# zilliztech/knowhere

Measured on AMD Instinct MI355X. Metric: QPS at recall@10>=0.95, IVF-PQ 100M x d=128 batch=10k, higher is better.
Workload: dtype f32

## Files before the change

include/knhip.h:

```cpp
#ifndef KNHIP_H
#define KNHIP_H

#include <stddef.h>
#include <stdint.h>

#ifdef __cplusplus
extern "C" {
#endif

#define KNHIP_ABI_VERSION 9

typedef struct knhip_index knhip_index;

typedef enum knhip_kind {
    KNHIP_BRUTE_FORCE = 0,
    KNHIP_IVF_FLAT = 1,
    KNHIP_IVF_PQ = 2,
    KNHIP_IVF_SQ8 = 3
} knhip_kind;

typedef enum knhip_metric { KNHIP_L2 = 0, KNHIP_IP = 1 } knhip_metric;

typedef enum knhip_status {
    KNHIP_OK = 0,
// ... 225 lines not shown
enum {
    KNHIP_STAGE_COARSE = 0,
    KNHIP_STAGE_GROUP = 1,
    KNHIP_STAGE_LUT = 2,
    KNHIP_STAGE_SCAN = 3,
    KNHIP_STAGE_MERGE = 4,
    KNHIP_STAGE_OTHER = 5,
    KNHIP_STAGE_SCAN_RANK0 = 6,
    KNHIP_STAGE_TABLES = 7,
    KNHIP_STAGE_REFINE = 8,
    KNHIP_STAGE_TIES = 9
};
int knhip_profile_enable(knhip_index* idx, int on);
int knhip_profile_reset(knhip_index* idx);
int knhip_profile_get(const knhip_index* idx, knhip_stage_times* out);
const char* knhip_stage_kernel_name(int stage, int kind);

#ifdef __cplusplus
}
#endif
#endif
```

knowhere_amd/_lib.py:

```python
import ctypes as C
import os

_HERE = os.path.dirname(os.path.abspath(__file__))
LIB_PATH = os.environ.get("KNHIP_LIB") or os.path.join(_HERE, "libknhip.so")

BRUTE_FORCE, IVF_FLAT, IVF_PQ, IVF_SQ8 = 0, 1, 2, 3
L2, IP = 0, 1
NSTAGE = 16
ABI_VERSION = 9
(STAGE_COARSE, STAGE_GROUP, STAGE_LUT, STAGE_SCAN, STAGE_MERGE, STAGE_OTHER, STAGE_SCAN_RANK0, STAGE_TABLES, STAGE_REFINE,
 STAGE_TIES) = range(10)
STAGE_NAMES = ["coarse", "group", "lut", "scan", "merge", "other", "scan_rank0", "tables", "refine", "ties"]


class KnhipError(RuntimeError):
    def __init__(self, code, msg):
        super().__init__(f"knhip error {code}: {msg}")
        self.code = code


class Desc(C.Structure):
    _fields_ = [("kind", C.c_int32), ("metric", C.c_int32), ("dim", C.c_int32), ("device", C.c_int32),
                ("nlist", C.c_int64), ("pq_m", C.c_int32), ("pq_nbits", C.c_int32),
                ("precomputed_table_max_bytes", C.c_int64)]


class StageTimes(C.Structure):
    _fields_ = [("ms", C.c_float * NSTAGE), ("launches", C.c_int64 * NSTAGE), ("scan_bytes", C.c_double),
                ("coarse_flops", C.c_double), ("scan_items", C.c_int64), ("coarse_fallback_queries", C.c_int64), ("scan_bytes_rank0", C.c_double),
                ("mscan_queries", C.c_int64), ("mscan_overflow_queries", C.c_int64), ("mscan_candidates", C.c_int64), ("mscan_stream_bytes", C.c_double),
                ("mscan_recomputed", C.c_int64), ("pq_filter_form", C.c_int64), ("tie_queries", C.c_int64),
                ("tie_anomalies", C.c_int64)]


SYMBOLS = [
    "knhip_abi_version", "knhip_device_count", "knhip_last_error", "knhip_index_create",
    "knhip_index_destroy", "knhip_index_set_coarse", "knhip_index_set_pq", "knhip_index_set_sq", "knhip_index_set_sq_type", "knhip_index_get_sq_type", "knhip_index_set_row_scale", "knhip_index_add_assigned_by", "knhip_index_get_desc",
    "knhip_index_add_lists", "knhip_index_add_vectors", "knhip_index_set_coarse_device",
    "knhip_index_set_lists_device", "knhip_index_add_vectors_device", "knhip_index_count",
    "knhip_index_device_bytes", "knhip_index_uses_precomputed_table", "knhip_index_last_range_ranks", "knhip_search",
    "knhip_search_device", "knhip_coarse_search_device", "knhip_merge_topk_device",
    "knhip_search_canonical_device", "knhip_ties_rule_applies", "knhip_tie_flag_device", "knhip_tie_arrivals_device", "knhip_tie_resolve_device",
    "knhip_tie_flag_host", "knhip_tie_resolve_host", "knhip_refine_distances_device", "knhip_refine_rows_distances_device",
    "knhip_refine_combine_device", "knhip_refine_select_device", "knhip_refine_select_host",
    "knhip_merge_topk_host", "knhip_refine_device", "knhip_fvec_L2sqr_ny", "knhip_fvec_inner_products_ny",
    "knhip_fvec_norms_L2sqr", "knhip_fvec_madd", "knhip_int8_vec_L2sqr_ny",
    "knhip_int8_vec_inner_products_ny", "knhip_profile_enable", "knhip_profile_reset",
    "knhip_profile_get", "knhip_stage_kernel_name", "knhip_range_search", "knhip_range_search_ranked", "knhip_free", "knhip_search_preassigned_device",
    "knhip_kmeans_device", "knhip_index_train", "knhip_index_train_device", "knhip_index_add", "knhip_index_add_device",
    "knhip_index_encode_device", "knhip_index_get_coarse", "knhip_index_get_pq", "knhip_index_get_sq",
    "knhip_index_get_list_sizes", "knhip_index_get_lists", "knhip_index_get_vectors_device", "knhip_search_refine",
    "knhip_index_get_vectors", "knhip_index_find_vectors", "knhip_index_assign", "knhip_device_memory",
    "knhip_rows_create", "knhip_rows_destroy", "knhip_rows_train", "knhip_rows_train_uniform", "knhip_rows_set_trained", "knhip_rows_get_trained",
    "knhip_rows_add", "knhip_rows_add_codes", "knhip_rows_get_codes", "knhip_rows_count", "knhip_rows_code_size",
    "knhip_rows_device_bytes", "knhip_search_refine_rows", "knhip_refine_rows_device",
# ... 58 lines not shown
    L.knhip_index_set_sq.argtypes = [vp, vp, vp]
    L.knhip_index_set_sq_type.argtypes = [vp, i32]
    L.knhip_index_get_sq_type.argtypes = [vp]
    L.knhip_index_get_sq_type.restype = i32
    L.knhip_index_set_row_scale.argtypes = [vp, vp, i32]
    L.knhip_index_add_assigned_by.argtypes = [vp, i64, vp, vp, vp]
    L.knhip_index_add_lists.argtypes = [vp, vp, vp, vp]
    L.knhip_index_set_lists_device.argtypes = [vp, vp, vp, vp]
    L.knhip_index_add_vectors.argtypes = [vp, i64, vp, vp, i64]
    L.knhip_index_add_vectors_device.argtypes = [vp, i64, vp, vp, i64]
    L.knhip_index_count.argtypes = [vp]
    L.knhip_index_device_bytes.argtypes = [vp]
    L.knhip_index_uses_precomputed_table.argtypes = [vp]
    L.knhip_index_last_range_ranks.argtypes = [vp]
    L.knhip_index_last_range_ranks.restype = C.c_int64
    L.knhip_search.argtypes = [vp, vp, i64, i32, i32, vp, i64, vp, vp]
    L.knhip_search_device.argtypes = [vp, vp, i64, i32, i32, vp, i64, vp, vp, vp]
    L.knhip_coarse_search_device.argtypes = [vp, vp, i64, i32, vp, vp, vp]
    L.knhip_search_preassigned_device.argtypes = [vp, vp, i64, i32, i32, vp, vp, vp, i64, vp, vp, vp]
    L.knhip_merge_topk_device.argtypes = [i32, i64, i32, i32, vp, vp, vp, vp, vp]
    L.knhip_merge_topk_host.argtypes = [i32, i64, i32, i32, vp, vp, vp, vp]
    L.knhip_refine_device.argtypes = [i32, i32, vp, i64, i64, vp, i64, vp, i32, i32, vp, vp, vp]
    L.knhip_search_canonical_device.argtypes = [vp, vp, i64, i32, i32, vp, vp, vp, i64, vp, vp, vp]
    L.knhip_tie_flag_device.argtypes = [vp, vp, i64, i32, vp, vp, vp, C.POINTER(C.c_int32), vp]
    L.knhip_tie_arrivals_device.argtypes = [vp, vp, vp, i32, vp, i32, i32, vp, vp, vp, i64, i64, vp, vp, vp, vp, vp]
    L.knhip_tie_resolve_device.argtypes = [i32, i32, vp, i32, i32, vp, vp, vp, vp, vp, vp, vp, vp, vp]
    L.knhip_tie_flag_host.argtypes = [vp, vp, i64, i32, vp, vp, vp]
    L.knhip_tie_resolve_host.argtypes = [i32, i32, i64, i32, vp, vp, vp, vp, vp, vp, vp, vp, vp]
    L.knhip_refine_distances_device.argtypes = [i32, i32, vp, i64, i64, vp, i64, vp, i32, vp, vp]
    L.knhip_refine_rows_distances_device.argtypes = [i32, vp, i64, vp, i64, vp, i32, vp, vp]
# ... 64 lines not shown
```

knowhere_amd/csrc/kernels.h:

```cpp
#pragma once

#include <hip/hip_runtime.h>
#include <stdint.h>
#include <algorithm>
#include "sq_codec.h"

namespace knhip {

struct KnItem {
    int32_t list;
    int32_t npair;
    int64_t pair0;
};
struct KnPair {
    int32_t q;
    int32_t slot;
};

__host__ __device__ constexpr int pq_stream_phase(int lane) {
    const int l = lane & 31;
    return l < 4 ? l : l < 12 ? l + 4 : l < 16 ? l - 8 : l < 20 ? l - 16 : l < 28 ? l - 12 : l - 24;
}
constexpr int PQ_STREAM_PHASES = 16;
__host__ __device__ constexpr uint32_t pq_stream_mask(int j) {
// ... 198 lines not shown
    const uint4* pq_codes_i;
    const void* pq_qi;
    const float* pq_qis;
    P16Rec* pq_recs16;
    int32_t* pq_ctr;
    int32_t pq_prune_mu;
    const void* pq_cb16;
    const void* pq_qh16;
    const float* pq_qd;
    const float* pq_sc;
    const float* pq_psum_s;
    unsigned char* pq_spill;
    int32_t pq_spill_cap;
    int32_t pq_spill_wgs;
    const int2* pq_unit_tiles;
};

int64_t pq_stream16r_blocks(int64_t len);
hipError_t launch_pq_stream16r(const uint8_t* codes, const int64_t* list_row_off, const int64_t* list_len,
                               const int64_t* list_sblk_off, int64_t nlist, uint4* out, hipStream_t s);
hipError_t launch_pq_psum(const uint8_t* codes, const int64_t* list_row_off, const int64_t* list_len,
                          const int64_t* list_sblk_off, int64_t nlist, const float* precomp_t, float* psum,
                          uint32_t* pabs_max_bits, hipStream_t s);
hipError_t launch_pqf_query_table(const float* queries, const float4* cb_m, int d, int64_t nq, bool is_l2, float pabs_max,
                                  void* qh, float* qs, hipStream_t s);
hipError_t launch_pqf_predict(const float* dump, int64_t stride, const int32_t* n_row, const float* gthr, const float* qs,
                              const float* qs2, const int64_t* keys, int nprobe, int64_t nlist, const int64_t* list_len,
                              int64_t nq, int cap, int k, bool is_l2, int32_t* poor, hipStream_t s);
size_t pqf_smem();
hipError_t launch_pq_stream16i(const uint8_t* codes, const int64_t* list_row_off, const int64_t* list_len,
// ... 79 lines not shown
    return std::max<int64_t>(groups, std::min<int64_t>(by_cost, by_tiles));
}
hipError_t launch_mscan_flat(const MScanArgs& a, bool is_l2, int64_t units_bound, hipStream_t s);
int mscan_flat_bf16_qt(int nstep);
size_t mscan_flat_bf16_smem(int nstep);
hipError_t launch_mscan_flat_bf16(const MScanArgs& a, bool is_l2, int64_t units_bound, hipStream_t s);
hipError_t launch_mscan_sq8(const MScanArgs& a, bool is_l2, int64_t units_bound, hipStream_t s);
hipError_t launch_ms_sample_plan(const int64_t* keys, int64_t nq, int nprobe, int64_t nlist, const int64_t* list_len,
                                 int smin, int cap, int32_t* sample_off, int32_t* n_row, hipStream_t s);
hipError_t launch_ms_sq8_query_prep(const float* queries, int64_t nq, int d, int ldq, const float* trained, void* qh,
                                    void* ql, float* qs, hipStream_t s, int bits = 8);
hipError_t launch_ms_tau(const float* sel_d, int64_t nq, int k, bool is_l2, float* gthr, uint2* gmeta, hipStream_t s);
hipError_t launch_mscan_finish(const MScanArgs& a, int kind, bool is_l2, const int64_t* keys, const float* coarse_dis,
                               int nprobe, int k, float* out_d, int64_t* out_i, unsigned long long* counters, int pass,
                               hipStream_t s);
hipError_t launch_ms_flag_pairs(const int32_t* overflow, int want, const int64_t* keys, int64_t nq, int nprobe,
                                int64_t nlist, const int64_t* list_len, int k, KnItem* items, KnPair* pairs,
                                int64_t* nitems, int64_t* empty_mark, hipStream_t s);

hipError_t launch_sq_scan(const SqScanArgs& a, bool is_l2, int64_t grid, hipStream_t s, int qg_override = 0);
hipError_t launch_sq_interleave(const uint8_t* codes, const int64_t* list_row_off,
                                const int64_t* list_len, const int64_t* list_blk_off, int64_t nlist,
                                int64_t code_size, uint4* out, hipStream_t s);

struct WorkTable {
    int32_t* list_count;
    int64_t* list_pair_off;
    int64_t* list_item_off;
    int32_t* list_cursor;
    KnPair* pairs;
// ... 204 lines not shown
```

knowhere_amd/csrc/knhip_api.hip:

```cpp
#include "knhip_internal.h"

namespace knhip_host {

thread_local std::string g_last_error;

int fail(int code, const std::string& msg) {
    g_last_error = msg;
    return code;
}

int build_coarse_layout(knhip_index* idx) {
    const int nchunk = (idx->d + 3) / 4;
    const int64_t nblk = (idx->nlist + 63) / 64;
    HIP_TRY(idx->centroids_il.alloc((size_t)nblk * nchunk * 64 * sizeof(float4)));
    HIP_TRY(launch_interleave_rows(idx->centroids.as<float>(), idx->nlist, idx->d,
                                   idx->centroids_il.as<float4>(), 0, nullptr));
    HIP_TRY(idx->cnorm.alloc((size_t)idx->nlist * sizeof(float)));
    HIP_TRY(launch_row_norms(idx->centroids.as<float>(), idx->nlist, idx->d, idx->cnorm.as<float>(), nullptr));
    HIP_TRY(idx->centroids_bs.alloc((size_t)idx->nlist * coarse_bf16_slabs(idx->d) * 128));
    HIP_TRY(launch_coarse_bf16_split(idx->centroids.as<float>(), idx->nlist, idx->d, idx->centroids_bs.p, nullptr));
    HIP_TRY(hipDeviceSynchronize());
    std::vector<float> cn((size_t)idx->nlist);
    HIP_TRY(hipMemcpy(cn.data(), idx->cnorm.p, cn.size() * sizeof(float), hipMemcpyDeviceToHost));
    idx->cnorm_max = cn.empty() ? 0.f : *std::max_element(cn.begin(), cn.end());
// ... 767 lines not shown
        }
        const int qt0 = mscan_queries_per_unit(kind, true);
        const int64_t units_bound = round_up(npairs / qt + std::min<int64_t>(nlist, npairs) + 1, 8);
        const int64_t sample = mscan_sample_rows();
        const int64_t np0 = std::min<int64_t>(npairs, nq * std::min<int64_t>(nprobe, sample));
        const int64_t bound0 = round_up(np0 / qt0 + std::min<int64_t>(nlist, np0) + 1, 8);
        HIP_TRY(ws->ms_units.reserve((size_t)std::max(units_bound, bound0) * sizeof(KnItem)));
        HIP_TRY(ws->ms_unit_off.reserve((size_t)(nlist + 1) * sizeof(int64_t)));
        HIP_TRY(ws->ms_nunits.reserve(sizeof(int64_t) + 2 * sizeof(double)));
        HIP_TRY(ws->ms_cand.reserve((size_t)nq * ms_cap * sizeof(int64_t)));
        HIP_TRY(ws->ms_cand_pess.reserve((size_t)nq * ms_cap * sizeof(float)));
        if (kind == KNHIP_IVF_SQ8) {
            HIP_TRY(ws->ms_eps_max.reserve((size_t)nq * sizeof(uint32_t)));
            HIP_TRY(hipMemsetAsync(ws->ms_eps_max.p, 0, (size_t)nq * sizeof(uint32_t), s));
        }
        HIP_TRY(ws->ms_cand_cnt.reserve((size_t)(2 * nq + 4) * sizeof(int32_t)));
        HIP_TRY(ws->dump.reserve((size_t)nq * sample * sizeof(float)));
        HIP_TRY(ws->sel_keys.reserve((size_t)nq * k * sizeof(int64_t)));
        HIP_TRY(ws->sel_d.reserve((size_t)nq * k * sizeof(float)));
        HIP_TRY(ws->ghist.reserve((size_t)nq * 64 * sizeof(uint32_t)));
        HIP_TRY(ws->gmeta.reserve((size_t)nq * sizeof(uint2)));
        int32_t* cand_cnt = ws->ms_cand_cnt.as<int32_t>();
        int32_t* overflow = cand_cnt + nq;
        MScanArgs m{};
        m.rows = idx->rows.p;
        m.xnorm = idx->xnorm.as<float>();
        m.xnorm_max = idx->xnorm_max;
        m.list_blk_off = idx->d_list_blk_off.as<int64_t>();
        m.list_len = idx->d_list_len.as<int64_t>();
        m.list_row_off = idx->d_list_row_off.as<int64_t>();
        m.ids = idx->ids.as<int64_t>();
// ... 327 lines not shown
        {
            StageTimer t(idx, s, KNHIP_STAGE_SCAN);
            HIP_TRY(launch_filter(m, std::max(units_bound, pqd_bound)));
        }
        {
            StageTimer t(idx, s, KNHIP_STAGE_MERGE);
            unsigned long long* counters = idx->coarse_fail_dev.as<unsigned long long>() + 1;
            MScanArgs mf = m;
            if (pq_i8) {
                mf.pq_qs = m.pq_qis;
                mf.pq_prune_mu = 1;
            }
            if (pq_dec) {
                mf.pq_qs = m.pq_qd;
            }
            HIP_TRY(launch_mscan_finish(mf, kind, is_l2, keys_p, cdis_p, nprobe, k, d_out_d, d_out_i, counters, 1, s));
            HIP_TRY(launch_ms_flag_pairs(overflow, 2, keys_p, nq, nprobe, nlist, idx->d_list_len.as<int64_t>(), k,
                                         ws->items.as<KnItem>(), wt.pairs, wt.nitems, nullptr, s));
            MScanArgs r = m;
            r.pairs = wt.pairs;
            r.units = ws->items.as<KnItem>();
            r.nunits_dev = wt.nitems;
            r.unit_loop = 1;
            r.pq_unit_tiles = nullptr;
            r.ghist = nullptr;
            r.gmeta = nullptr;
            HIP_TRY(launch_filter(r, npairs));
            HIP_TRY(launch_mscan_finish(mf, kind, is_l2, keys_p, cdis_p, nprobe, k, d_out_d, d_out_i, counters, 2, s));
            HIP_TRY(launch_ms_flag_pairs(overflow, 1, keys_p, nq, nprobe, nlist, idx->d_list_len.as<int64_t>(), k,
                                         ws->items.as<KnItem>(), wt.pairs, wt.nitems, ws->partial_i.as<int64_t>(), s));
// ... 672 lines not shown
    if (!out) {
        return fail(KNHIP_ERR_INVALID_ARGS, "get_desc: null output");
    }
    *out = idx->desc;
    return KNHIP_OK;
}

int64_t knhip_index_device_bytes(const knhip_index* idx) {
    return idx ? idx->device_bytes() : 0;
}

int64_t knhip_index_last_range_ranks(const knhip_index* idx) {
    return idx ? idx->last_range_ranks : -1;
}

int knhip_index_uses_precomputed_table(const knhip_index* idx) {
    return idx ? idx->use_precomp : 0;
}


int knhip_search_device(const knhip_index* idx, const float* d_queries, int64_t nq, int32_t k,
                        int32_t nprobe, const uint8_t* d_bitset, int64_t bitset_nbits,
                        int64_t* d_out_ids, float* d_out_dist, void* stream) {
    if (int rc = check_index(idx)) return rc;
    if (int rc = validate_search(idx, nq, k, nprobe)) return rc;
    if (nq == 0) {
        return KNHIP_OK;
    }
    if (!d_queries || !d_out_ids || !d_out_dist) {
        return fail(KNHIP_ERR_INVALID_ARGS, "null query/output pointer");
// ... 717 lines not shown
```

knowhere_amd/csrc/knhip_env.h:

```cpp
#pragma once
#include <algorithm>
#include <cstdlib>
#include <cstring>

namespace knhip_host {

struct EnvLayout {
    bool coarse_given;
    int coarse_gemm;
    size_t aos_keep_bytes;
    bool rank0_select;
    bool cand_hist;
    int pq_q4;
    int mscan;
    bool flat_bf16;
    int mscan_cap;
    int pqd_spill_cap;
    int pqf;
    bool pqf_guard;
    int pqf_form;
    bool pq_v1;
    bool bf_exact;
    int pq_waves;
};

struct EnvSearch {
    int ms_sample_rows;
    int pq_sample_rows;
    bool no_side_stream;
    bool guard_sync;
    bool range_no_waves;
    bool ties_canonical;
    bool ties_trace;
    int pqd_unit_cost;
};
constexpr int KNHIP_PQD_UNIT_COST_DEFAULT = 512;

inline bool env_is(const char* v, const char* what) { return v != nullptr && std::strcmp(v, what) == 0; }
inline int env_digit(const char* v, int lo, int hi, int dflt) { return (v && v[0] >= '0' + lo && v[0] <= '0' + hi) ? v[0] - '0' : dflt; }
inline int env_count(const char* v) { return (v && *v) ? std::max(0, std::atoi(v)) : 0; }

inline EnvLayout env_layout() {
    EnvLayout e{};
    const char* c = std::getenv("KNHIP_COARSE");
    e.coarse_given = c != nullptr;
    e.coarse_gemm = env_is(c, "exact") ? 0 : env_is(c, "fp32") ? 1 : 2;
    const char* keep = std::getenv("KNHIP_AOS_KEEP_MB");
    e.aos_keep_bytes = (keep && *keep) ? (size_t)std::max<long long>(0, std::atoll(keep)) << 20 : (size_t)8 << 30;
    const char* r0 = std::getenv("KNHIP_RANK0");
// ... 21 lines not shown

inline EnvSearch env_search() {
    EnvSearch e{};
    const char* a = std::getenv("KNHIP_MS_SAMPLE_ROWS");
    e.ms_sample_rows = a ? std::max(1, std::atoi(a)) : 0;
    const char* b = std::getenv("KNHIP_PQ_SAMPLE_ROWS");
    e.pq_sample_rows = b ? std::max(1, std::atoi(b)) : 0;
    e.no_side_stream = std::getenv("KNHIP_NO_SIDE_STREAM") != nullptr;
    e.guard_sync = std::getenv("KNHIP_PQF_GUARD_SYNC") != nullptr;
    e.range_no_waves = std::getenv("KNHIP_RANGE_NO_WAVES") != nullptr;
    const char* t = std::getenv("KNHIP_TIES");
    e.ties_canonical = t && (t[0] == 'c' || t[0] == 'C' || t[0] == '0');
    e.ties_trace = std::getenv("KNHIP_TIES_TRACE") != nullptr;
    const char* uc = std::getenv("KNHIP_PQD_UNIT_COST");
    e.pqd_unit_cost = (uc && *uc) ? std::max(0, std::atoi(uc)) : KNHIP_PQD_UNIT_COST_DEFAULT;
    return e;
}

}
```

knowhere_amd/csrc/mfma_scan.hip:

```cpp
#include "common.h"
#include "kernels.h"
#include "ms_common.h"

namespace knhip {

typedef float ms_f32x16 __attribute__((ext_vector_type(16)));
typedef _Float16 ms_f16x8 __attribute__((ext_vector_type(8)));

constexpr int MS_WAVES = 4;
constexpr int MS_THREADS = MS_WAVES * KN_WAVE;
constexpr int MS_NQT = 2;
constexpr int MS_QT = 32 * MS_NQT;
constexpr int MS_SAMPLE = 8192;

__global__ void ms_block_norms_kernel(const float4* __restrict__ rows, int64_t total_blk, int nchunk,
                                      float* __restrict__ out, float* __restrict__ out_max) {
    const int64_t t = (int64_t)blockIdx.x * blockDim.x + threadIdx.x;
    float acc = 0.f;
    if (t < total_blk * 64) {
        const int64_t b = t >> 6;
        const int r = (int)(t & 63);
        const float4* p = rows + b * (int64_t)nchunk * 64 + r;
        for (int c = 0; c < nchunk; c++) {
            const float4 v = p[(int64_t)c * 64];
// ... 964 lines not shown
        return hipSuccess;
    }
    if (is_l2) {
        hipLaunchKernelGGL(ms_tau_kernel<true>, dim3((unsigned)((nq + 255) / 256)), dim3(256), 0, s, sel_d, nq, k, gthr,
                           gmeta);
    } else {
        hipLaunchKernelGGL(ms_tau_kernel<false>, dim3((unsigned)((nq + 255) / 256)), dim3(256), 0, s, sel_d, nq, k, gthr,
                           gmeta);
    }
    return hipGetLastError();
}

constexpr int MF_THREADS = 256;
constexpr int MF_MLP = 8;

template <bool IS_L2, int KIND, int BITS = 8>
__global__ __launch_bounds__(MF_THREADS) void mscan_finish_kernel(MScanArgs a, const int64_t* __restrict__ keys,
                                                                  const float* __restrict__ coarse_dis, int nprobe,
                                                                  int k, int P_max, float* __restrict__ out_d,
                                                                  int64_t* __restrict__ out_i,
                                                                  unsigned long long* __restrict__ counters, int pass) {
    extern __shared__ __align__(16) unsigned char smem[];
    __shared__ float tab[256];
    static_assert(KIND == 3 || BITS == 8, "the code width belongs to the IVF-SQ finish");
    const int64_t q = blockIdx.x;
    const int tid = threadIdx.x;
    const int flag = a.overflow[q];
    const bool retry_prep = pass == 1 && flag == 1;
    if ((pass == 1 && flag != 0 && flag != 1) || (pass == 2 && flag != 2)) {
        if (pass == 2 && flag == 1 && tid == 0) {
            atomicAdd(counters + 1, 1ull);
        }
        return;
    }
    const int d = a.d;
    int n = min(a.cand_cnt[q], a.cap);
    const int n_filter = n;
    constexpr int MF_PRUNE_PER_THREAD = 16;
    const int n_head = min(n, MF_THREADS * MF_PRUNE_PER_THREAD);
    if ((KIND != 3 || a.eps_max != nullptr) && a.cand_pess != nullptr && !retry_prep && n >= 2 * k &&
        n_head <= MF_THREADS * MF_PRUNE_PER_THREAD) {
        __shared__ int s_cnt;
        __shared__ float s_red[MF_THREADS / KN_WAVE];
        float cmax = 0.f;
        for (int sl = tid; KIND == 2 && sl < nprobe; sl += MF_THREADS) {
            cmax = fmaxf(cmax, fabsf(coarse_dis[q * nprobe + sl]));
        }
#pragma unroll
        for (int dlt = KN_WAVE / 2; dlt > 0; dlt >>= 1) {
// ... 75 lines not shown
                if (tot >= k) {
                    hi = mid;
                } else {
                    lo = mid + 1;
                }
            }
        }
        const float tau2 = dist_key_inv<IS_L2>(lo);
        float tau_abs = fmaxf(gthr_abs, fabsf(tau2));
        if (KIND == 2 && n_head < n && a.gmeta != nullptr) {
            const uint2 mt = a.gmeta[q];
            if (mt.y != KN_HIST_OFF) {
                tau_abs = fmaxf(tau_abs, fabsf(dist_key_inv<IS_L2>(mt.x)));
            }
        }
        float eps_max = eps_q + 64.0f * 5.9604645e-8f * (cmax + tau_abs + eps_mu);
        if (KIND == 1) {
            const float qn = a.qnorm[q];
            eps_max = a.eps_scale * (IS_L2 ? (qn + a.xnorm_max) : sqrtf(qn * a.xnorm_max)) + 1e-30f;
        }
        if (KIND == 3) {
            eps_max = __uint_as_float(a.eps_max[q]);
        }
        if (eps_max < INFINITY && tau2 == tau2 && fabsf(tau2) < FLT_MAX) {
            if (tid == 0) {
                s_cnt = 0;
            }
            __syncthreads();
#pragma unroll
            for (int u = 0; u < MF_PRUNE_PER_THREAD; u++) {
                const int ci = tid + u * MF_THREADS;
                const bool keep = ci < n_head && (IS_L2 ? (pp[u] - 2.0f * eps_max <= tau2) : (pp[u] + 2.0f * eps_max >= tau2));
                if (keep) {
                    const int j = atomicAdd(&s_cnt, 1);
                    a.cand[q * (int64_t)a.cap + j] = pc[u];
                }
            }
#pragma unroll 1
            for (int ci0 = n_head; ci0 < n; ci0 += MF_THREADS) {
                const int ci = ci0 + tid;
                int64_t c = 0;
                float p = worst_dist<IS_L2>();
                if (ci < n) {
                    c = a.cand[q * (int64_t)a.cap + ci];
                    p = a.cand_pess[q * (int64_t)a.cap + ci];
                }
                __syncthreads();
                if (ci < n && (IS_L2 ? (p - 2.0f * eps_max <= tau2) : (p + 2.0f * eps_max >= tau2))) {
                    const int j = atomicAdd(&s_cnt, 1);
                    a.cand[q * (int64_t)a.cap + j] = c;
                }
            }
            __syncthreads();
            n = s_cnt;
            __syncthreads();
        }
    }
    if (retry_prep && n < k) {
        if (tid == 0) {
            atomicAdd(counters + 1, 1ull);
            a.overflow[q] = 3;
        }
        return;
// ... 62 lines not shown
                                    acc = l2_step(acc, x.x, y.x);
                                    acc = l2_step(acc, x.y, y.y);
                                    acc = l2_step(acc, x.z, y.z);
                                    acc = l2_step(acc, x.w, y.w);
                                } else {
                                    acc = ip_step(acc, x.x, y.x);
                                    acc = ip_step(acc, x.y, y.y);
                                    acc = ip_step(acc, x.z, y.z);
                                    acc = ip_step(acc, x.w, y.w);
                                }
                            }
                        }
                    }
                } else if (KIND == 2) {
                    const uint4* cp = reinterpret_cast<const uint4*>(a.pq_codes + (a.list_row_off[list] + pos) * 32);
                    const uint4 cw[2] = {cp[0], cp[1]};
                    const uint32_t ww[8] = {cw[0].x, cw[0].y, cw[0].z, cw[0].w, cw[1].x, cw[1].y, cw[1].z, cw[1].w};
                    const float* cen = a.centroids + list * d;
#pragma unroll 16
                    for (int m = 0; m < 32; m++) {
                        const int code = (int)((ww[m >> 2] >> (8 * (m & 3))) & 0xffu);
                        const float4 y = a.pq_cb_t[code * 32 + m];
                        float4 x = *reinterpret_cast<const float4*>(sq + m * 4);
                        float t;
                        if (a.pq_lut_mode == PQ_LUT_RESIDUAL) {
                            const float4 cl = *reinterpret_cast<const float4*>(cen + m * 4);
                            x = make_float4(fsub_x(x.x, cl.x), fsub_x(x.y, cl.y), fsub_x(x.z, cl.z), fsub_x(x.w, cl.w));
                            t = l2_step(0.f, x.x, y.x);
                            t = l2_step(t, x.y, y.y);
                            t = l2_step(t, x.z, y.z);
                            t = l2_step(t, x.w, y.w);
                        } else {
                            t = ip_step(0.f, x.x, y.x);
                            t = ip_step(t, x.y, y.y);
                            t = ip_step(t, x.z, y.z);
                            t = ip_step(t, x.w, y.w);
                            if (a.pq_lut_mode == PQ_LUT_PRECOMP) {
                                const float4 cl = *reinterpret_cast<const float4*>(cen + m * 4);
                                float nrm = ip_step(0.f, y.x, y.x);
                                nrm = ip_step(nrm, y.y, y.y);
                                nrm = ip_step(nrm, y.z, y.z);
                                nrm = ip_step(nrm, y.w, y.w);
                                float ipc = ip_step(0.f, cl.x, y.x);
                                ipc = ip_step(ipc, cl.y, y.y);
                                ipc = ip_step(ipc, cl.z, y.z);
                                ipc = ip_step(ipc, cl.w, y.w);
                                const float t2 = fadd_x(nrm, fmul_x(2.0f, ipc));
                                t = fadd_x(t2, fmul_x(-2.0f, t));
                            }
                        }
                        acc = fadd_x(acc, t);
                    }
                    if (a.pq_lut_mode != PQ_LUT_RESIDUAL) {
                        acc = fadd_x(coarse_dis[q * nprobe + slot], acc);
                    }
                } else if (BITS != 8) {
                    constexpr int GC = SW::GROUP_CHUNKS, GD = SW::GROUP_DIMS;
                    constexpr int NG = BITS == 6 ? 2 : 4;
                    const uint4* p = reinterpret_cast<const uint4*>(a.rows) + blk * (int64_t)a.nchunk * 64 + r;
                    const float* cen = a.centroids + list * d;
                    for (int g0 = 0; g0 < sq_ngroup; g0 += NG) {
                        uint4 wv[NG * GC];
#pragma unroll
                        for (int u = 0; u < NG * GC; u++) {
                            wv[u] = p[(int64_t)min(g0 * GC + u, a.nchunk - 1) * 64];
                        }
#pragma unroll
                        for (int gu = 0; gu < NG; gu++) {
                            const int g = g0 + gu;
                            if (g < sq_ngroup) {
// ... 98 lines not shown
        }
        return;
    }
    for (int e = tid; e < k; e += MF_THREADS) {
        float dd = worst_dist<IS_L2>();
        int64_t ii = -1;
        if (!(key[e] == 0xffffffffu && tie[e] == ~0ull)) {
            dd = dist_key_inv<IS_L2>(key[e]);
            ii = (int64_t)(IS_L2 ? tie[e] : ~tie[e]);
        }
        out_d[q * k + e] = dd;
        out_i[q * k + e] = ii;
    }
    if (pass == 2 && tid == 0) {
        a.overflow[q] = 0;
    }
}

__global__ void ms_flag_pairs_kernel(const int32_t* __restrict__ overflow, int want, const int64_t* __restrict__ keys,
                                     int64_t nq, int nprobe, int64_t nlist, const int64_t* __restrict__ list_len, int k,
                                     KnItem* __restrict__ items, KnPair* __restrict__ pairs, int64_t* __restrict__ nitems,
                                     int64_t* __restrict__ empty_mark) {
    if (overflow[nq] == 0) {
        return;
    }
    const int64_t t = (int64_t)blockIdx.x * blockDim.x + threadIdx.x;
    if (t >= nq * nprobe) {
        return;
    }
    const int64_t q = t / nprobe;
// ... 136 lines not shown
    if (kind == 1) {
        if (is_l2) MF_LAUNCH(true, 1); else MF_LAUNCH(false, 1);
    } else if (kind == 2) {
        if (is_l2) MF_LAUNCH(true, 2); else MF_LAUNCH(false, 2);
    } else if (bits == 8) {
        if (is_l2) MF_LAUNCH(true, 3); else MF_LAUNCH(false, 3);
    } else if (bits == 6) {
        if (is_l2) MF_LAUNCH(true, 3, 6); else MF_LAUNCH(false, 3, 6);
    } else {
        if (is_l2) MF_LAUNCH(true, 3, 4); else MF_LAUNCH(false, 3, 4);
    }
#undef MF_LAUNCH
    return hipGetLastError();
}

}
```

knowhere_amd/index.py:

```python
import ctypes as C

import numpy as np

from . import _lib
from ._lib import KnhipError, check

BRUTE_FORCE, IVF_FLAT, IVF_PQ, IVF_SQ8 = _lib.BRUTE_FORCE, _lib.IVF_FLAT, _lib.IVF_PQ, _lib.IVF_SQ8
L2, IP = _lib.L2, _lib.IP

KIND_NAMES = {"GPU_HIP_BRUTE_FORCE": BRUTE_FORCE, "GPU_HIP_IVF_FLAT": IVF_FLAT, "GPU_HIP_IVF_PQ": IVF_PQ,
              "GPU_HIP_IVF_SQ8": IVF_SQ8}


def _np_ptr(a):
    return None if a is None else C.c_void_p(a.ctypes.data)


def _t_ptr(t):
    return None if t is None else C.c_void_p(t.data_ptr())


def _bitset_nbits(bitset, nbits):
    if bitset is None:
        return 0
# ... 208 lines not shown
        I = np.empty((nq, k), np.int64)
        bs = None if bitset is None else np.ascontiguousarray(bitset, np.uint8)
        nbits = _bitset_nbits(bs, nbits)
        check(self.L.knhip_search_refine_rows(self.h, rows.h, _np_ptr(xq), nq, k, k_base, nprobe, _np_ptr(bs), nbits,
                                              _np_ptr(I), _np_ptr(D)))
        return D, I

    def get_vectors(self, ids):
        ids = np.ascontiguousarray(ids, np.int64)
        out = np.empty((len(ids), self.dim), np.float32)
        check(self.L.knhip_index_get_vectors(self.h, len(ids), _np_ptr(ids), _np_ptr(out)))
        return out

    def last_range_ranks(self):
        return int(self.L.knhip_index_last_range_ranks(self.h))

    def range_search(self, xq, radius, max_empty_result_buckets=2, bitset=None, nbits=0):
        xq = np.ascontiguousarray(xq, np.float32)
        nq = xq.shape[0]
        lims = np.zeros(nq + 1, np.int64)
        pi, pd = C.POINTER(C.c_int64)(), C.POINTER(C.c_float)()
        bs = None if bitset is None else np.ascontiguousarray(bitset, np.uint8)
        nbits = _bitset_nbits(bs, nbits)
        check(self.L.knhip_range_search(self.h, _np_ptr(xq), nq, float(radius), int(max_empty_result_buckets),
                                        _np_ptr(bs), nbits, _np_ptr(lims), C.byref(pi), C.byref(pd)))
        n = int(lims[-1])
        ids = np.ctypeslib.as_array(pi, shape=(n,)).copy() if n else np.empty(0, np.int64)
        dis = np.ctypeslib.as_array(pd, shape=(n,)).copy() if n else np.empty(0, np.float32)
        self.L.knhip_free(pi)
        self.L.knhip_free(pd)
# ... 348 lines not shown
```

Before: 1.564 million.

## Add wave-per-query PQ finish kernel ahead of block finish pass

Adds a new finish kernel for IVF-PQ in which each 64-lane wave handles one query. It does ballot-based threshold pruning, exact PQ recomputation of the survivors and a rank-based top-k, all inside the wave. Queries it completes are marked done, and the existing block-per-query finish kernel skips them. The aim is to stop spending a whole 256-thread block and block-level syncs on queries with few candidates. The cost is an extra launch plus a fallback path for queries that overflow the wave kernel's limits.

Result: slower. 1.492 million (-4.6%).

```diff
diff --git a/include/knhip.h b/include/knhip.h
--- a/include/knhip.h
+++ b/include/knhip.h
@@ -263,6 +263,7 @@
 int knhip_profile_enable(knhip_index* idx, int on);
 int knhip_profile_reset(knhip_index* idx);
 int knhip_profile_get(const knhip_index* idx, knhip_stage_times* out);
+int64_t knhip_index_finish_wave_queries(const knhip_index* idx);
 const char* knhip_stage_kernel_name(int stage, int kind);
 
 #ifdef __cplusplus
diff --git a/knowhere_amd/_lib.py b/knowhere_amd/_lib.py
--- a/knowhere_amd/_lib.py
+++ b/knowhere_amd/_lib.py
@@ -38,7 +38,7 @@
     "knhip_index_destroy", "knhip_index_set_coarse", "knhip_index_set_pq", "knhip_index_set_sq", "knhip_index_set_sq_type", "knhip_index_get_sq_type", "knhip_index_set_row_scale", "knhip_index_add_assigned_by", "knhip_index_get_desc",
     "knhip_index_add_lists", "knhip_index_add_vectors", "knhip_index_set_coarse_device",
     "knhip_index_set_lists_device", "knhip_index_add_vectors_device", "knhip_index_count",
-    "knhip_index_device_bytes", "knhip_index_uses_precomputed_table", "knhip_index_last_range_ranks", "knhip_search",
+    "knhip_index_device_bytes", "knhip_index_uses_precomputed_table", "knhip_index_last_range_ranks", "knhip_index_finish_wave_queries", "knhip_search",
     "knhip_search_device", "knhip_coarse_search_device", "knhip_merge_topk_device",
     "knhip_search_canonical_device", "knhip_ties_rule_applies", "knhip_tie_flag_device", "knhip_tie_arrivals_device", "knhip_tie_resolve_device",
     "knhip_tie_flag_host", "knhip_tie_resolve_host", "knhip_refine_distances_device", "knhip_refine_rows_distances_device",
@@ -127,6 +127,8 @@
     L.knhip_index_uses_precomputed_table.argtypes = [vp]
     L.knhip_index_last_range_ranks.argtypes = [vp]
     L.knhip_index_last_range_ranks.restype = C.c_int64
+    L.knhip_index_finish_wave_queries.argtypes = [vp]
+    L.knhip_index_finish_wave_queries.restype = C.c_int64
     L.knhip_search.argtypes = [vp, vp, i64, i32, i32, vp, i64, vp, vp]
     L.knhip_search_device.argtypes = [vp, vp, i64, i32, i32, vp, i64, vp, vp, vp]
     L.knhip_coarse_search_device.argtypes = [vp, vp, i64, i32, vp, vp, vp]
diff --git a/knowhere_amd/csrc/kernels.h b/knowhere_amd/csrc/kernels.h
--- a/knowhere_amd/csrc/kernels.h
+++ b/knowhere_amd/csrc/kernels.h
@@ -236,6 +236,7 @@
     int32_t pq_spill_cap;
     int32_t pq_spill_wgs;
     const int2* pq_unit_tiles;
+    const int32_t* finish_done;
 };
 
 int64_t pq_stream16r_blocks(int64_t len);
@@ -345,6 +346,10 @@
 hipError_t launch_mscan_finish(const MScanArgs& a, int kind, bool is_l2, const int64_t* keys, const float* coarse_dis,
                                int nprobe, int k, float* out_d, int64_t* out_i, unsigned long long* counters, int pass,
                                hipStream_t s);
+bool mscan_finish_wave_supports(const MScanArgs& a, int kind, int k);
+hipError_t launch_mscan_finish_wave(const MScanArgs& a, int kind, bool is_l2, const int64_t* keys,
+                                    const float* coarse_dis, int nprobe, int k, float* out_d, int64_t* out_i,
+                                    unsigned long long* counters, int32_t* done, hipStream_t s);
 hipError_t launch_ms_flag_pairs(const int32_t* overflow, int want, const int64_t* keys, int64_t nq, int nprobe,
                                 int64_t nlist, const int64_t* list_len, int k, KnItem* items, KnPair* pairs,
                                 int64_t* nitems, int64_t* empty_mark, hipStream_t s);
diff --git a/knowhere_amd/csrc/knhip_api.hip b/knowhere_amd/csrc/knhip_api.hip
--- a/knowhere_amd/csrc/knhip_api.hip
+++ b/knowhere_amd/csrc/knhip_api.hip
@@ -805,7 +805,7 @@
             HIP_TRY(ws->ms_eps_max.reserve((size_t)nq * sizeof(uint32_t)));
             HIP_TRY(hipMemsetAsync(ws->ms_eps_max.p, 0, (size_t)nq * sizeof(uint32_t), s));
         }
-        HIP_TRY(ws->ms_cand_cnt.reserve((size_t)(2 * nq + 4) * sizeof(int32_t)));
+        HIP_TRY(ws->ms_cand_cnt.reserve((size_t)(3 * nq + 4) * sizeof(int32_t)));
         HIP_TRY(ws->dump.reserve((size_t)nq * sample * sizeof(float)));
         HIP_TRY(ws->sel_keys.reserve((size_t)nq * k * sizeof(int64_t)));
         HIP_TRY(ws->sel_d.reserve((size_t)nq * k * sizeof(float)));
@@ -1163,6 +1163,12 @@
             if (pq_dec) {
                 mf.pq_qs = m.pq_qd;
             }
+            if (!env.finish_block && mscan_finish_wave_supports(mf, kind, k)) {
+                int32_t* done = ws->ms_cand_cnt.as<int32_t>() + 2 * nq + 4;
+                HIP_TRY(launch_mscan_finish_wave(mf, kind, is_l2, keys_p, cdis_p, nprobe, k, d_out_d, d_out_i, counters,
+                                                 done, s));
+                mf.finish_done = done;
+            }
             HIP_TRY(launch_mscan_finish(mf, kind, is_l2, keys_p, cdis_p, nprobe, k, d_out_d, d_out_i, counters, 1, s));
             HIP_TRY(launch_ms_flag_pairs(overflow, 2, keys_p, nq, nprobe, nlist, idx->d_list_len.as<int64_t>(), k,
                                          ws->items.as<KnItem>(), wt.pairs, wt.nitems, nullptr, s));
@@ -1865,6 +1871,19 @@
     return idx ? idx->last_range_ranks : -1;
 }
 
+int64_t knhip_index_finish_wave_queries(const knhip_index* idx) {
+    if (check_index(idx) != KNHIP_OK) {
+        return -1;
+    }
+    DeviceGuard g(idx->desc.device);
+    unsigned long long n = 0;
+    if (hipDeviceSynchronize() != hipSuccess ||
+        hipMemcpy(&n, idx->coarse_fail_dev.as<unsigned long long>() + 6, sizeof(n), hipMemcpyDeviceToHost) != hipSuccess) {
+        return -1;
+    }
+    return (int64_t)n;
+}
+
 int knhip_index_uses_precomputed_table(const knhip_index* idx) {
     return idx ? idx->use_precomp : 0;
 }
diff --git a/knowhere_amd/csrc/knhip_env.h b/knowhere_amd/csrc/knhip_env.h
--- a/knowhere_amd/csrc/knhip_env.h
+++ b/knowhere_amd/csrc/knhip_env.h
@@ -33,6 +33,7 @@
     bool ties_canonical;
     bool ties_trace;
     int pqd_unit_cost;
+    bool finish_block;
 };
 constexpr int KNHIP_PQD_UNIT_COST_DEFAULT = 512;
 
@@ -84,6 +85,7 @@
     e.ties_trace = std::getenv("KNHIP_TIES_TRACE") != nullptr;
     const char* uc = std::getenv("KNHIP_PQD_UNIT_COST");
     e.pqd_unit_cost = (uc && *uc) ? std::max(0, std::atoi(uc)) : KNHIP_PQD_UNIT_COST_DEFAULT;
+    e.finish_block = env_is(std::getenv("KNHIP_FINISH"), "block");
     return e;
 }
 
diff --git a/knowhere_amd/csrc/mfma_scan.hip b/knowhere_amd/csrc/mfma_scan.hip
--- a/knowhere_amd/csrc/mfma_scan.hip
+++ b/knowhere_amd/csrc/mfma_scan.hip
@@ -1002,6 +1002,58 @@
 constexpr int MF_THREADS = 256;
 constexpr int MF_MLP = 8;
 
+__device__ __forceinline__ float mf_pq_exact(const MScanArgs& a, const float* sq, const uint4 cw0, const uint4 cw1,
+                                             const float* __restrict__ cen, const float* __restrict__ cd) {
+    const uint32_t ww[8] = {cw0.x, cw0.y, cw0.z, cw0.w, cw1.x, cw1.y, cw1.z, cw1.w};
+    float acc = 0.f;
+#pragma unroll 16
+    for (int m = 0; m < 32; m++) {
+        const int code = (int)((ww[m >> 2] >> (8 * (m & 3))) & 0xffu);
+        const float4 y = a.pq_cb_t[code * 32 + m];
+        float4 x = *reinterpret_cast<const float4*>(sq + m * 4);
+        float t;
+        if (a.pq_lut_mode == PQ_LUT_RESIDUAL) {
+            const float4 cl = *reinterpret_cast<const float4*>(cen + m * 4);
+            x = make_float4(fsub_x(x.x, cl.x), fsub_x(x.y, cl.y), fsub_x(x.z, cl.z), fsub_x(x.w, cl.w));
+            t = l2_step(0.f, x.x, y.x);
+            t = l2_step(t, x.y, y.y);
+            t = l2_step(t, x.z, y.z);
+            t = l2_step(t, x.w, y.w);
+        } else {
+            t = ip_step(0.f, x.x, y.x);
+            t = ip_step(t, x.y, y.y);
+            t = ip_step(t, x.z, y.z);
+            t = ip_step(t, x.w, y.w);
+            if (a.pq_lut_mode == PQ_LUT_PRECOMP) {
+                const float4 cl = *reinterpret_cast<const float4*>(cen + m * 4);
+                float nrm = ip_step(0.f, y.x, y.x);
+                nrm = ip_step(nrm, y.y, y.y);
+                nrm = ip_step(nrm, y.z, y.z);
+                nrm = ip_step(nrm, y.w, y.w);
+                float ipc = ip_step(0.f, cl.x, y.x);
+                ipc = ip_step(ipc, cl.y, y.y);
+                ipc = ip_step(ipc, cl.z, y.z);
+                ipc = ip_step(ipc, cl.w, y.w);
+                const float t2 = fadd_x(nrm, fmul_x(2.0f, ipc));
+                t = fadd_x(t2, fmul_x(-2.0f, t));
+            }
+        }
+        acc = fadd_x(acc, t);
+    }
+    if (a.pq_lut_mode != PQ_LUT_RESIDUAL) {
+        acc = fadd_x(*cd, acc);
+    }
+    return acc;
+}
+
+__device__ __forceinline__ float mf_pq_eps_max(float eps_q, float cmax, float tau_abs, float eps_mu) {
+    return eps_q + 64.0f * 5.9604645e-8f * (cmax + tau_abs + eps_mu);
+}
+template <bool IS_L2>
+__device__ __forceinline__ bool mf_prune_keep(float p, float eps_max, float tau2) {
+    return IS_L2 ? (p - 2.0f * eps_max <= tau2) : (p + 2.0f * eps_max >= tau2);
+}
+
 template <bool IS_L2, int KIND, int BITS = 8>
 __global__ __launch_bounds__(MF_THREADS) void mscan_finish_kernel(MScanArgs a, const int64_t* __restrict__ keys,
                                                                   const float* __restrict__ coarse_dis, int nprobe,
@@ -1021,6 +1073,9 @@
         }
         return;
     }
+    if (pass == 1 && a.finish_done != nullptr && a.finish_done[q] != 0) {
+        return;
+    }
     const int d = a.d;
     int n = min(a.cand_cnt[q], a.cap);
     const int n_filter = n;
@@ -1126,7 +1181,7 @@
                 tau_abs = fmaxf(tau_abs, fabsf(dist_key_inv<IS_L2>(mt.x)));
             }
         }
-        float eps_max = eps_q + 64.0f * 5.9604645e-8f * (cmax + tau_abs + eps_mu);
+        float eps_max = mf_pq_eps_max(eps_q, cmax, tau_abs, eps_mu);
         if (KIND == 1) {
             const float qn = a.qnorm[q];
             eps_max = a.eps_scale * (IS_L2 ? (qn + a.xnorm_max) : sqrtf(qn * a.xnorm_max)) + 1e-30f;
@@ -1142,7 +1197,7 @@
 #pragma unroll
             for (int u = 0; u < MF_PRUNE_PER_THREAD; u++) {
                 const int ci = tid + u * MF_THREADS;
-                const bool keep = ci < n_head && (IS_L2 ? (pp[u] - 2.0f * eps_max <= tau2) : (pp[u] + 2.0f * eps_max >= tau2));
+                const bool keep = ci < n_head && mf_prune_keep<IS_L2>(pp[u], eps_max, tau2);
                 if (keep) {
                     const int j = atomicAdd(&s_cnt, 1);
                     a.cand[q * (int64_t)a.cap + j] = pc[u];
@@ -1158,7 +1213,7 @@
                     p = a.cand_pess[q * (int64_t)a.cap + ci];
                 }
                 __syncthreads();
-                if (ci < n && (IS_L2 ? (p - 2.0f * eps_max <= tau2) : (p + 2.0f * eps_max >= tau2))) {
+                if (ci < n && mf_prune_keep<IS_L2>(p, eps_max, tau2)) {
                     const int j = atomicAdd(&s_cnt, 1);
                     a.cand[q * (int64_t)a.cap + j] = c;
                 }
@@ -1251,46 +1306,7 @@
                     }
                 } else if (KIND == 2) {
                     const uint4* cp = reinterpret_cast<const uint4*>(a.pq_codes + (a.list_row_off[list] + pos) * 32);
-                    const uint4 cw[2] = {cp[0], cp[1]};
-                    const uint32_t ww[8] = {cw[0].x, cw[0].y, cw[0].z, cw[0].w, cw[1].x, cw[1].y, cw[1].z, cw[1].w};
-                    const float* cen = a.centroids + list * d;
-#pragma unroll 16
-                    for (int m = 0; m < 32; m++) {
-                        const int code = (int)((ww[m >> 2] >> (8 * (m & 3))) & 0xffu);
-                        const float4 y = a.pq_cb_t[code * 32 + m];
-                        float4 x = *reinterpret_cast<const float4*>(sq + m * 4);
-                        float t;
-                        if (a.pq_lut_mode == PQ_LUT_RESIDUAL) {
-                            const float4 cl = *reinterpret_cast<const float4*>(cen + m * 4);
-                            x = make_float4(fsub_x(x.x, cl.x), fsub_x(x.y, cl.y), fsub_x(x.z, cl.z), fsub_x(x.w, cl.w));
-                            t = l2_step(0.f, x.x, y.x);
-                            t = l2_step(t, x.y, y.y);
-                            t = l2_step(t, x.z, y.z);
-                            t = l2_step(t, x.w, y.w);
-                        } else {
-                            t = ip_step(0.f, x.x, y.x);
-                            t = ip_step(t, x.y, y.y);
-                            t = ip_step(t, x.z, y.z);
-                            t = ip_step(t, x.w, y.w);
-                            if (a.pq_lut_mode == PQ_LUT_PRECOMP) {
-                                const float4 cl = *reinterpret_cast<const float4*>(cen + m * 4);
-                                float nrm = ip_step(0.f, y.x, y.x);
-                                nrm = ip_step(nrm, y.y, y.y);
-                                nrm = ip_step(nrm, y.z, y.z);
-                                nrm = ip_step(nrm, y.w, y.w);
-                                float ipc = ip_step(0.f, cl.x, y.x);
-                                ipc = ip_step(ipc, cl.y, y.y);
-                                ipc = ip_step(ipc, cl.z, y.z);
-                                ipc = ip_step(ipc, cl.w, y.w);
-                                const float t2 = fadd_x(nrm, fmul_x(2.0f, ipc));
-                                t = fadd_x(t2, fmul_x(-2.0f, t));
-                            }
-                        }
-                        acc = fadd_x(acc, t);
-                    }
-                    if (a.pq_lut_mode != PQ_LUT_RESIDUAL) {
-                        acc = fadd_x(coarse_dis[q * nprobe + slot], acc);
-                    }
+                    acc = mf_pq_exact(a, sq, cp[0], cp[1], a.centroids + list * d, coarse_dis + q * nprobe + slot);
                 } else if (BITS != 8) {
                     constexpr int GC = SW::GROUP_CHUNKS, GD = SW::GROUP_DIMS;
                     constexpr int NG = BITS == 6 ? 2 : 4;
@@ -1419,6 +1435,232 @@
     }
     if (pass == 2 && tid == 0) {
         a.overflow[q] = 0;
+    }
+}
+
+constexpr int MFW_WAVES = 4;
+constexpr int MFW_PER_LANE = 16;
+constexpr int MFW_MAX_N = KN_WAVE * MFW_PER_LANE;
+constexpr int MFW_MAX_K = 128;
+constexpr int MFW_MAX_SURV = 256;
+constexpr int MFW_DQ = 128;
+constexpr int MFW_LDS_WAVE = MFW_MAX_SURV * 12 + MFW_DQ * 4;
+
+__device__ __forceinline__ void mfw_wave_sync() {
+    __builtin_amdgcn_fence(__ATOMIC_RELEASE, "wavefront");
+    __builtin_amdgcn_wave_barrier();
+    __builtin_amdgcn_fence(__ATOMIC_ACQUIRE, "wavefront");
+}
+
+template <bool IS_L2, int KIND>
+__global__ __launch_bounds__(MFW_WAVES * KN_WAVE, 4) void mscan_finish_wave_kernel(
+    MScanArgs a, const int64_t* __restrict__ keys, const float* __restrict__ coarse_dis, int nprobe, int k,
+    float* __restrict__ out_d, int64_t* __restrict__ out_i, unsigned long long* __restrict__ counters,
+    int32_t* __restrict__ done) {
+    extern __shared__ __align__(16) unsigned char smem[];
+    static_assert(KIND == 2, "the wave finish recomputes PQ codes; the other kinds stay on the block kernel");
+    const int lane = threadIdx.x & (KN_WAVE - 1);
+    const int wave = __builtin_amdgcn_readfirstlane((int)(threadIdx.x / KN_WAVE));
+    const int64_t q = (int64_t)blockIdx.x * MFW_WAVES + wave;
+    if (q >= a.nq) {
+        return;
+    }
+    const int n = min(a.cand_cnt[q], a.cap);
+    if (a.overflow[q] != 0 || n > MFW_MAX_N) {
+        if (lane == 0) {
+            done[q] = 0;
+        }
+        return;
+    }
+    unsigned char* my = smem + (size_t)wave * MFW_LDS_WAVE;
+    unsigned long long* tie = reinterpret_cast<unsigned long long*>(my);
+    uint32_t* key = reinterpret_cast<uint32_t*>(my + MFW_MAX_SURV * 8);
+    float* sq = reinterpret_cast<float*>(my + MFW_MAX_SURV * 12);
+    const int d = a.d;
+    for (int i = lane; i < MFW_DQ; i += KN_WAVE) {
+        sq[i] = (i < d) ? a.queries[q * d + i] : 0.f;
+    }
+    const bool have_pess = a.cand_pess != nullptr;
+    int64_t pc[MFW_PER_LANE];
+    float pp[MFW_PER_LANE];
+#pragma unroll
+    for (int u = 0; u < MFW_PER_LANE; u++) {
+        const int ci = lane + u * KN_WAVE;
+        pc[u] = 0;
+        pp[u] = worst_dist<IS_L2>();
+        if (u * KN_WAVE < n && ci < n) {
+            pc[u] = a.cand[q * (int64_t)a.cap + ci];
+            if (have_pess) {
+                pp[u] = a.cand_pess[q * (int64_t)a.cap + ci];
+            }
+        }
+    }
+    bool pruned = false;
+    float tau2 = 0.f, eps_max = 0.f;
+    if (have_pess && n >= 2 * k) {
+        float cmax = 0.f;
+        for (int sl = lane; sl < nprobe; sl += KN_WAVE) {
+            cmax = fmaxf(cmax, fabsf(coarse_dis[q * nprobe + sl]));
+        }
+        uint32_t kmn = 0xffffffffu, kmx = 0u;
+#pragma unroll
+        for (int u = 0; u < MFW_PER_LANE; u++) {
+            if (lane + u * KN_WAVE < n) {
+                const uint32_t pk = dist_key<IS_L2>(pp[u]);
+                kmn = min(kmn, pk);
+                kmx = max(kmx, pk);
+            }
+        }
+#pragma unroll
+        for (int dlt = KN_WAVE / 2; dlt > 0; dlt >>= 1) {
+            cmax = fmaxf(cmax, __shfl_xor(cmax, dlt, KN_WAVE));
+            kmn = min(kmn, (uint32_t)__shfl_xor((int)kmn, dlt, KN_WAVE));
+            kmx = max(kmx, (uint32_t)__shfl_xor((int)kmx, dlt, KN_WAVE));
+        }
+        uint32_t lo = kmn, hi = kmx;
+        while (lo < hi) {
+            const uint32_t mid = lo + ((hi - lo) >> 1);
+            int c = 0;
+#pragma unroll
+            for (int u = 0; u < MFW_PER_LANE; u++) {
+                if (u * KN_WAVE < n) {
+                    c += __popcll(__ballot(lane + u * KN_WAVE < n && dist_key<IS_L2>(pp[u]) <= mid));
+                }
+            }
+            if (c >= k) {
+                hi = mid;
+            } else {
+                lo = mid + 1;
+            }
+        }
+        tau2 = dist_key_inv<IS_L2>(lo);
+        const float eps_q = a.pq_qs[q * 4 + 2];
+        const float eps_mu = a.pq_prune_mu ? fabsf(a.pq_qs[q * 4 + 1]) : 0.f;
+        const float tau_abs = fmaxf(fabsf(a.gthr[q]), fabsf(tau2));
+        eps_max = mf_pq_eps_max(eps_q, cmax, tau_abs, eps_mu);
+        pruned = eps_max < INFINITY && tau2 == tau2 && fabsf(tau2) < FLT_MAX;
+    }
+    uint32_t keepbits = 0;
+    int ns = 0;
+#pragma unroll
+    for (int u = 0; u < MFW_PER_LANE; u++) {
+        if (u * KN_WAVE < n) {
+            const bool keep = lane + u * KN_WAVE < n && (!pruned || mf_prune_keep<IS_L2>(pp[u], eps_max, tau2));
+            keepbits |= keep ? (1u << u) : 0u;
+            ns += __popcll(__ballot(keep));
+        }
+    }
+    if (ns > MFW_MAX_SURV) {
+        if (lane == 0) {
+            done[q] = 0;
+        }
+        return;
+    }
+    {
+        const unsigned long long below = (1ull << lane) - 1ull;
+        int base = 0;
+#pragma unroll
+        for (int u = 0; u < MFW_PER_LANE; u++) {
+            if (u * KN_WAVE < n) {
+                const bool keep = (keepbits >> u) & 1u;
+                const unsigned long long b = __ballot(keep);
+                if (keep) {
+                    tie[base + __popcll(b & below)] = (unsigned long long)pc[u];
+                }
+                base += __popcll(b);
+            }
+        }
+    }
+    mfw_wave_sync();
+    const bool add_coarse = a.pq_lut_mode != PQ_LUT_RESIDUAL;
+#pragma unroll 1
+    for (int b0 = 0; b0 < ns; b0 += 2 * KN_WAVE) {
+        int slot[2];
+        int64_t pos[2], list[2], row[2], id[2];
+        float cdv[2];
+        uint4 cw[2][2];
+#pragma unroll
+        for (int r = 0; r < 2; r++) {
+            const unsigned long long c = tie[min(b0 + r * KN_WAVE + lane, ns - 1)];
+            slot[r] = (int)(c >> 32);
+            pos[r] = (int64_t)(uint32_t)c;
+        }
+        mfw_wave_sync();
+#pragma unroll
+        for (int r = 0; r < 2; r++) {
+            list[r] = keys[q * nprobe + slot[r]];
+            cdv[r] = add_coarse ? coarse_dis[q * nprobe + slot[r]] : 0.f;
+        }
+#pragma unroll
+        for (int r = 0; r < 2; r++) {
+            row[r] = a.list_row_off[list[r]] + pos[r];
+        }
+#pragma unroll
+        for (int r = 0; r < 2; r++) {
+            const uint4* cp = reinterpret_cast<const uint4*>(a.pq_codes + row[r] * 32);
+            cw[r][0] = cp[0];
+            cw[r][1] = cp[1];
+            id[r] = a.ids[row[r]];
+        }
+#pragma unroll
+        for (int r = 0; r < 2; r++) {
+            if (b0 + r * KN_WAVE < ns) {
+                const float acc = mf_pq_exact(a, sq, cw[r][0], cw[r][1], a.centroids + list[r] * d, &cdv[r]);
+                const int j = b0 + r * KN_WAVE + lane;
+                if (j < ns) {
+                    key[j] = dist_key<IS_L2>(acc);
+                    tie[j] = IS_L2 ? (unsigned long long)id[r] : ~(unsigned long long)id[r];
+                }
+            }
+        }
+    }
+    mfw_wave_sync();
+    constexpr int NR = MFW_MAX_SURV / KN_WAVE;
+    uint32_t mk[NR];
+    unsigned long long mt[NR];
+    int rank[NR];
+#pragma unroll
+    for (int r = 0; r < NR; r++) {
+        const int j = min(r * KN_WAVE + lane, max(ns - 1, 0));
+        mk[r] = key[j];
+        mt[r] = tie[j];
+        rank[r] = 0;
+    }
+#pragma unroll 2
+    for (int i = 0; i < ns; i++) {
+        const uint32_t ki = key[i];
+        const unsigned long long ti = tie[i];
+#pragma unroll
+        for (int r = 0; r < NR; r++) {
+            if (r * KN_WAVE < ns) {
+                const bool less = ki < mk[r] || (ki == mk[r] && (ti < mt[r] || (ti == mt[r] && i < r * KN_WAVE + lane)));
+                rank[r] += less ? 1 : 0;
+            }
+        }
+    }
+#pragma unroll
+    for (int r = 0; r < NR; r++) {
+        if (r * KN_WAVE + lane < ns && rank[r] < k) {
+            float dd = worst_dist<IS_L2>();
+            int64_t ii = -1;
+            if (!(mk[r] == 0xffffffffu && mt[r] == ~0ull)) {
+                dd = dist_key_inv<IS_L2>(mk[r]);
+                ii = (int64_t)(IS_L2 ? mt[r] : ~mt[r]);
+            }
+            out_d[q * k + rank[r]] = dd;
+            out_i[q * k + rank[r]] = ii;
+        }
+    }
+    for (int e = ns + lane; e < k; e += KN_WAVE) {
+        out_d[q * k + e] = worst_dist<IS_L2>();
+        out_i[q * k + e] = -1;
+    }
+    if (lane == 0) {
+        atomicAdd(counters, 1ull);
+        atomicAdd(counters + 2, (unsigned long long)n);
+        atomicAdd(counters + 3, (unsigned long long)ns);
+        atomicAdd(counters + 5, 1ull);
+        done[q] = 1;
     }
 }
 
@@ -1585,4 +1827,30 @@
     return hipGetLastError();
 }
 
-}
+
+bool mscan_finish_wave_supports(const MScanArgs& a, int kind, int k) {
+    return kind == 2 && k >= 1 && k <= MFW_MAX_K && a.nchunk * 4 == MFW_DQ && a.d <= MFW_DQ;
+}
+
+hipError_t launch_mscan_finish_wave(const MScanArgs& a, int kind, bool is_l2, const int64_t* keys,
+                                    const float* coarse_dis, int nprobe, int k, float* out_d, int64_t* out_i,
+                                    unsigned long long* counters, int32_t* done, hipStream_t s) {
+    if (a.nq <= 0) {
+        return hipSuccess;
+    }
+    if (!mscan_finish_wave_supports(a, kind, k) || done == nullptr) {
+        return hipErrorInvalidValue;
+    }
+    const unsigned grid = (unsigned)((a.nq + MFW_WAVES - 1) / MFW_WAVES);
+    const size_t sm = (size_t)MFW_WAVES * MFW_LDS_WAVE;
+    if (is_l2) {
+        hipLaunchKernelGGL((mscan_finish_wave_kernel<true, 2>), dim3(grid), dim3(MFW_WAVES * KN_WAVE), sm, s, a, keys,
+                           coarse_dis, nprobe, k, out_d, out_i, counters, done);
+    } else {
+        hipLaunchKernelGGL((mscan_finish_wave_kernel<false, 2>), dim3(grid), dim3(MFW_WAVES * KN_WAVE), sm, s, a, keys,
+                           coarse_dis, nprobe, k, out_d, out_i, counters, done);
+    }
+    return hipGetLastError();
+}
+
+}
diff --git a/knowhere_amd/index.py b/knowhere_amd/index.py
--- a/knowhere_amd/index.py
+++ b/knowhere_amd/index.py
@@ -246,6 +246,9 @@
 
     def last_range_ranks(self):
         return int(self.L.knhip_index_last_range_ranks(self.h))
+
+    def finish_wave_queries(self):
+        return int(self.L.knhip_index_finish_wave_queries(self.h))
 
     def range_search(self, xq, radius, max_empty_result_buckets=2, bitset=None, nbits=0):
         xq = np.ascontiguousarray(xq, np.float32)
```
